# edantec/MPC_benchmark

Hardware: AMD Instinct MI355X
Metric: mpc_solves_per_sec (higher is better)
Workload: dtype f64

## Files before the change

### mpc_benchmark_amd/csrc/legs.h

```cpp
#pragma once
#include "mfma_blocks.h"
#include "solver_kernels.h"

#define LEG_BARRIER() asm volatile("s_waitcnt lgkmcnt(0)\n\ts_barrier" ::: "memory")

#define LEG_LAUNDER() do { asm volatile("" : "+v"(tid), "+v"(lane)); wv = __builtin_amdgcn_readfirstlane(tid >> 6); } while (0)

#define LK_THREADS 512
#define LK_U 20
#define LK_PT 13
#define LK_TILES 5

struct LkLds {
  int np, mp, nzp, lda, ldp, ldm, nb, nbm;
  int AB, PR, TM, ZN, vec, total_bytes;
  unsigned mg_nzp, mg_np, mg_mp;
};
static inline constexpr LkLds make_lk_lds(int n, int m) {
  LkLds s{};
  s.np = (n + 15) & ~15; s.mp = (m + 15) & ~15; s.nzp = s.np + s.mp; s.lda = s.nzp + 1; s.ldp = s.np + 1; s.ldm = s.mp + 1;
  s.nb = s.np / 16; s.nbm = s.mp / 16;
  s.mg_nzp = magic_div(s.nzp); s.mg_np = magic_div(s.np); s.mg_mp = magic_div(s.mp);
  int o = 0;
  auto take = [&](int cnt) { int r = o; o += (cnt + 1) & ~1; return r; };
// ... 733 lines not shown
  constexpr int FW_ROWS = NP / 8;
  for (int j = 0; j + 1 < J; ++j) {
    double* lr = leg_ptr(a, b, j);
    const int cut = leg_start(a, j + 1);
    const int c0 = lane < n ? lane : 0, c1 = lane + 64 < n ? lane + 64 : 0;
    const double m0 = lane < n ? 1.0 : 0.0, m1 = lane + 64 < n ? 1.0 : 0.0;
    double va[FW_ROWS][2];
    if (j > 0) {
#pragma unroll
      for (int i = 0; i < FW_ROWS; ++i) { const int r = wv + i * nw, rr = r < n ? r : 0; va[i][0] = lr[L.lZx + rr * n + c0] * m0; va[i][1] = lr[L.lZx + rr * n + c1] * m1; }
    }
#pragma unroll
    for (int i = 0; i < FW_ROWS; ++i) {
      const int r = wv + i * nw;
      double sx = 0.0;
      if (j > 0) sx = wave_sum(va[i][0] * xv[c0] + va[i][1] * xv[c1]);
      if (lane == 0 && r < n) { ev[r] = sx + lr[L.lzc + r]; a.dxs[((size_t)b * (N + 1) + cut) * n + r] = ev[r]; }
    }
#pragma unroll
    for (int i = 0; i < FW_ROWS; ++i) { const int r = wv + i * nw, rr = r < n ? r : 0; va[i][0] = lr[L.ldP + rr * n + c0] * m0; va[i][1] = lr[L.ldP + rr * n + c1] * m1; }
    LEG_BARRIER();
#pragma unroll
    for (int i = 0; i < FW_ROWS; ++i) {
      const int r = wv + i * nw;
      const double sx = wave_sum(va[i][0] * ev[c0] + va[i][1] * ev[c1]);
      if (lane == 0 && r < n) lr[L.lth + r] = sx + lr[L.lcp + r];
    }
    for (int i = tid; i < n; i += nthr) xv[i] = ev[i];
    LEG_BARRIER();
  }
  LEG_PROF(29);
}

__global__ void __launch_bounds__(256) k_leg_apply(SolverArgs a) {
  const Layout& L = a.L;
  const int k = blockIdx.x, b = blockIdx.y, tid = threadIdx.x, nthr = blockDim.x, lane = tid & 63, wv = tid >> 6, nw = nthr >> 6;
  const InstState& st = a.inst[b];
  if (st.done || st.skip_step) return;
  const int j = leg_of_knot(a, k);
  if (j + 1 >= a.nlegs) return;
  const int n = L.n, ke = leg_start(a, j + 1) - 1;
  const double* kn = knot_ptr(a, b, k);
  double* g = gain_ptr(a, b, k);
  const int m = (int)kn[L.oMISC + MISC_M], c = (int)kn[L.oMISC + MISC_NC];
  const double* th_g = leg_ptr(a, b, j) + L.lth;
  __shared__ double th[128], pn[128];
  __shared__ int act_idx[256];
  __shared__ int wcnt[4];
  for (int i = tid; i < n; i += nthr) th[i] = th_g[i];
  const bool is_act = tid < c && kn[L.oACT + (tid < c ? tid : 0)] != 0.0;
  const unsigned long long amask = __ballot(is_act);
  if (lane == 0) wcnt[wv] = __popcll(amask);
  __syncthreads();
  int ca = 0;
  {
    int off = 0;
    for (int q = 0; q < nw; ++q) { if (q < wv) off += wcnt[q]; ca += wcnt[q]; }
    if (is_act) act_idx[off + __popcll(amask & ((1ull << lane) - 1ull))] = tid;
  }
  const int c0 = lane < n ? lane : 0, c1 = lane + 64 < n ? lane + 64 : 0;
  const double m0 = lane < n ? 1.0 : 0.0, m1 = lane + 64 < n ? 1.0 : 0.0;
  if (k == ke) { for (int i = tid; i < n; i += nthr) pn[i] = th[i]; }
  else {
    const double* gn = gain_ptr(a, b, k + 1) + L.oLm;
    const double t0 = th[c0] * m0, t1 = th[c1] * m1;
    for (int r0 = 4 * wv; r0 < n; r0 += 4 * nw) {
      double v[4][2];
#pragma unroll
      for (int q = 0; q < 4; ++q) { const int r = r0 + q < n ? r0 + q : 0; v[q][0] = gn[r * n + c0]; v[q][1] = gn[r * n + c1]; }
#pragma unroll
      for (int q = 0; q < 4; ++q) { const double sx = wave_sum(v[q][0] * t0 + v[q][1] * t1); if (lane == 0 && r0 + q < n) pn[r0 + q] = sx; }
    }
  }
  __syncthreads();
  const double t0 = th[c0] * m0, t1 = th[c1] * m1, q0 = pn[c0] * m0, q1 = pn[c1] * m1;
  const int total = 2 * n + m + ca;
  for (int r0 = 4 * wv; r0 < total; r0 += 4 * nw) {
    double v[4][2];
    double* dst[4];
    bool use_th[4];
#pragma unroll
    for (int q = 0; q < 4; ++q) {
      const int r = r0 + q < total ? r0 + q : 0;
      const double* row;
      if (r < n) { row = g + L.oLm + r * n; dst[q] = g + L.op + r; use_th[q] = true; }
      else if (r < 2 * n) { row = g + L.oGam + (r - n) * n; dst[q] = g + L.ophi + (r - n); use_th[q] = false; }
      else if (r < 2 * n + m) { row = g + L.oKu + (r - 2 * n) * n; dst[q] = g + L.ok + (r - 2 * n); use_th[q] = false; }
      else { row = g + L.oKnup + (r - 2 * n - m) * n; dst[q] = g + L.oknu + act_idx[r - 2 * n - m]; use_th[q] = false; }
      v[q][0] = row[c0]; v[q][1] = row[c1];
    }
#pragma unroll
    for (int q = 0; q < 4; ++q) {
      const double sx = wave_sum(use_th[q] ? v[q][0] * t0 + v[q][1] * t1 : v[q][0] * q0 + v[q][1] * q1);
      if (lane == 0 && r0 + q < total) *dst[q] += sx;
    }
  }
}
```

### mpc_benchmark_amd/csrc/mpc_hip.hip

```cpp
#include <hip/hip_runtime.h>
#include <mutex>
#include <map>
#include <cmath>
#include <cstdio>
#include <cstdlib>
#include <cstring>
#include <limits>
#include <stdexcept>
#include <string>
#include <utility>
#include <vector>

#include "eval_multibody_host.h"
#include "eval_reuse_kernels.h"
#include "eval_vector.h"
#include "riccati_mfma.h"
#include "closed_loop.h"
#include "legs.h"
#include "legs_tree.h"
#include "pipeline_glue.h"
#include "pipeline_ikid_glue.h"
#include "pipeline_contacts.h"
#include "pipeline_fd_glue.h"
#include "sim_record.h"
// ... 134 lines not shown
  size_t d_patch_cap = 0;
  double* h_xnext[2] = {nullptr, nullptr};
  std::vector<double> leg_mu;
  static constexpr int ASYNC_DEPTH = 2;
  InstState* h_status[ASYNC_DEPTH] = {nullptr, nullptr};
  hipEvent_t status_ev[ASYNC_DEPTH] = {nullptr, nullptr};
  int async_head = 0, async_pending = 0;
  static constexpr int STAGE_RING = 8;
  char* stage_pin[STAGE_RING] = {};
  hipEvent_t stage_ev[STAGE_RING] = {};
  int stage_next = 0;
  RicLds ric{};
  int ric_fixed = 0;
  ClLds cl{};
  bool use_mfma_riccati = false;
  LkLds lk{};
  LcLds lc{};
  LxLds lx{};
  bool legs_ok = false;
  bool env_chain = false, env_plain = false, env_reject_failed = false;
  int env_tree_sweeps = 0, env_trace = -1;
  int env_tail_knots = -1, cu_count = 0;
  int tail_last = 0, tail_sweeps_last = 0;
  long long tail_fused = 0, tail_separate = 0;
  long long leg_passes_multi = 0, leg_passes_single = 0;
  int leg_tail_knots(int J) const {
    if (J < 2 || env_tail_knots == 0) return 0;
    const int last = L.N - (int)((long long)(J - 1) * L.N / J);
    if (env_tail_knots > 0) return env_tail_knots < last ? env_tail_knots : last;
    if ((long long)J * L.B > cu_count || (long long)L.N * L.B <= cu_count) return 0;
    const int t = 21 * (L.N / J) / 25;
    return t < last ? t : last;
  }
  double* d_legbuf = nullptr;
  double* d_treebuf = nullptr;
  int leg_cap = 0;
  TreeDesc tree{};
  bool use_tree() const {
    return eff_legs() >= 3 && d_treebuf != nullptr && !env_chain;
  }
  bool leg_guess_valid = false;
  int leg_guess_now = 0;
  int eff_legs() const {
    if (!legs_ok) return 1;
    int J = opt.riccati_legs;
    if (J > MPC_MAX_LEGS) J = MPC_MAX_LEGS;
    if (J > L.N) J = L.N;
    return J < 1 ? 1 : J;
  }
  struct ProfSlot {
    const char* name;
    std::vector<std::pair<hipEvent_t, hipEvent_t>> ev;
    size_t used = 0;
  };
  bool profiling = false;
  unsigned prof_mask = ~0u;
  std::vector<ProfSlot> prof;

  template <class F> void timed(int slot, const char* name, F&& launch) {
    if (!profiling || !((prof_mask >> slot) & 1u) || pass_is_corrector) { launch(); return; }
    if ((int)prof.size() <= slot) prof.resize(slot + 1);
    ProfSlot& p = prof[slot];
    p.name = name;
    if (p.used == p.ev.size()) {
      hipEvent_t e0, e1;
      HIP_OK(hipEventCreate(&e0));
// ... 48 lines not shown
}

static void ensure_leg_capacity(mpc_solver* s, int legs) {
  const Layout& L = s->L;
  int need = legs < 1 ? 1 : legs;
  if (need >= 3 && need < 4) need = 4;
  if (need <= s->leg_cap) return;
  HIP_OK(hipStreamSynchronize(s->stream));
  auto regrow = [&](double*& p, size_t count) {
    if (p) HIP_OK(hipFree(p));
    p = nullptr;
    HIP_OK(hipMalloc((void**)&p, (count ? count : 1) * sizeof(double)));
    HIP_OK(hipMemsetAsync(p, 0, (count ? count : 1) * sizeof(double), s->stream));
  };
  const size_t B = L.B;
  regrow(s->d_work, B * need * (size_t)L.work_stride);
  if (s->legs_ok) {
    regrow(s->d_legbuf, B * (size_t)(need > 1 ? need - 1 : 1) * L.leg_stride);
    regrow(s->d_treebuf, B * (size_t)need * L.tree_stride);
  }
  s->leg_cap = need;
  s->leg_guess_valid = false;
  HIP_OK(hipStreamSynchronize(s->stream));
}

static void create_impl(mpc_solver* s, const mpc_dims& d) {
  s->dims = d;
  { const char* e;
    e = getenv("MPC_LEGS_CHAIN"); s->env_chain = e && atoi(e) > 0;
    e = getenv("MPC_LEGS_PLAIN"); s->env_plain = e && atoi(e) > 0;
    e = getenv("MPC_HIP_REJECT_FAILED"); s->env_reject_failed = e && atoi(e) > 0;
    e = getenv("MPC_TREE_SWEEPS"); s->env_tree_sweeps = e ? atoi(e) : 0;
    e = getenv("MPC_HIP_TRACE"); s->env_trace = e ? atoi(e) : -1;
    e = getenv("MPC_LEG_TAIL_KNOTS"); s->env_tail_knots = e ? (atoi(e) > 0 ? atoi(e) : 0) : -1; }
  HIP_OK(hipSetDevice(d.device));
  HIP_OK(hipDeviceGetAttribute(&s->cu_count, hipDeviceAttributeMultiprocessorCount, d.device));
  { const char* e = getenv("MPC_LEG_TAIL_CUS"); if (e && atoi(e) > 0) s->cu_count = atoi(e); }
  {
    static int created = 0;
    const char* pe = getenv("MPC_HIP_STREAM_PRIO");
    if (pe && atoi(pe) > 0) {
      int lo = 0, hi = 0;
      HIP_OK(hipDeviceGetStreamPriorityRange(&lo, &hi));
      const int levels = lo - hi + 1;
      const int prio = hi + (created++ % levels);
      HIP_OK(hipStreamCreateWithPriority(&s->stream, hipStreamNonBlocking, prio));
      if (atoi(pe) > 1) fprintf(stderr, "[mpc] stream priority %d (range %d..%d)\n", prio, hi, lo);
    } else {
      HIP_OK(hipStreamCreateWithFlags(&s->stream, hipStreamNonBlocking));
    }
  }
  Layout& L = s->L;
  L.N = d.horizon; L.B = d.batch; L.space = d.space; L.nx = d.nx; L.n = d.ndx; L.m = d.nu; L.c = d.nc_max > 0 ? d.nc_max : 1;
  L.nj = 0;
  L.max_stage_ints = d.max_stage_ints; L.max_stage_doubles = d.max_stage_doubles;
  L.n_alpha = 8;
  make_layout(L);
  Layout& T = s->LT;
  T = L;
  {
    int o = 0;
    auto take = [&](int cnt) { int r = o; o += align2(cnt); return r; };
    T.oCV = take(L.c); T.oCT = take(L.c); T.oLO = take(L.c); T.oHI = take(L.c); T.oDT = take(L.c); T.oACT = take(L.c);
    T.oF = take(L.n); T.oMISC = take(MISC_COUNT);
    T.oH = T.oG = T.oAB = T.oE6 = T.oT6k = T.oD12 = T.oCD = T.oXD = T.oWR = T.oXN = 0;
    T.knot_stride = o;
  }
// ... 379 lines not shown
        case 48: MPC_TREE_LAUNCH(48); break;
        case 64: MPC_TREE_LAUNCH(64); break;
        default: MPC_TREE_LAUNCH(80); break;
      }
#undef MPC_TREE_LAUNCH
    });
    if (tree) s->timed(16, "k_leg_tree_down", [&] {
      const TreeDesc& T = s->tree;
      if (false) {
#define X(ID, FN, FM, GF, ST, NPV, MPV) } else if (s->ric_fixed == ID) { for (int lev = T.nlev - 1; lev >= 0; --lev) hipLaunchKernelGGL((k_leg_tree_down<NPV, FN, FM>), dim3(T.lev_cnt[lev] + (lev == T.nlev - 1 ? 1 : 0), L.B), dim3(LK_THREADS), s->lx.total_bytes, s->stream, a, s->lx, T, lev);
      MPC_FIXED_MODELS(X)
#undef X
      } else switch (s->lx.np) {
        case 16: for (int lev = T.nlev - 1; lev >= 0; --lev) hipLaunchKernelGGL(k_leg_tree_down<16>, dim3(T.lev_cnt[lev] + (lev == T.nlev - 1 ? 1 : 0), L.B), dim3(LK_THREADS), s->lx.total_bytes, s->stream, a, s->lx, T, lev); break;
        case 32: for (int lev = T.nlev - 1; lev >= 0; --lev) hipLaunchKernelGGL(k_leg_tree_down<32>, dim3(T.lev_cnt[lev] + (lev == T.nlev - 1 ? 1 : 0), L.B), dim3(LK_THREADS), s->lx.total_bytes, s->stream, a, s->lx, T, lev); break;
        case 48: for (int lev = T.nlev - 1; lev >= 0; --lev) hipLaunchKernelGGL(k_leg_tree_down<48>, dim3(T.lev_cnt[lev] + (lev == T.nlev - 1 ? 1 : 0), L.B), dim3(LK_THREADS), s->lx.total_bytes, s->stream, a, s->lx, T, lev); break;
        case 64: for (int lev = T.nlev - 1; lev >= 0; --lev) hipLaunchKernelGGL(k_leg_tree_down<64>, dim3(T.lev_cnt[lev] + (lev == T.nlev - 1 ? 1 : 0), L.B), dim3(LK_THREADS), s->lx.total_bytes, s->stream, a, s->lx, T, lev); break;
        default: for (int lev = T.nlev - 1; lev >= 0; --lev) hipLaunchKernelGGL(k_leg_tree_down<80>, dim3(T.lev_cnt[lev] + (lev == T.nlev - 1 ? 1 : 0), L.B), dim3(LK_THREADS), s->lx.total_bytes, s->stream, a, s->lx, T, lev); break;
      }
    });
    else s->timed(14, "k_leg_consensus", [&] {
      switch (s->lx.np) {
        case 16: hipLaunchKernelGGL(k_leg_consensus<16>, dim3(L.B), dim3(LK_THREADS), s->lx.total_bytes, s->stream, a, s->lx); break;
        case 32: hipLaunchKernelGGL(k_leg_consensus<32>, dim3(L.B), dim3(LK_THREADS), s->lx.total_bytes, s->stream, a, s->lx); break;
        case 48: hipLaunchKernelGGL(k_leg_consensus<48>, dim3(L.B), dim3(LK_THREADS), s->lx.total_bytes, s->stream, a, s->lx); break;
        case 64: hipLaunchKernelGGL(k_leg_consensus<64>, dim3(L.B), dim3(LK_THREADS), s->lx.total_bytes, s->stream, a, s->lx); break;
        default: hipLaunchKernelGGL(k_leg_consensus<80>, dim3(L.B), dim3(LK_THREADS), s->lx.total_bytes, s->stream, a, s->lx); break;
      }
    });
  }
  }
  if (J > 1) {
    s->leg_guess_valid = true;
    s->timed(15, "k_leg_apply", [&] { hipLaunchKernelGGL(k_leg_apply, dim3(L.N, L.B), dim3(256), 0, s->stream, a); });
    s->timed(4, "k_forward", [&] {
      if (L.m <= 32) hipLaunchKernelGGL((k_forward_phi<4, 10>), dim3(L.B * J), dim3(512), 2 * L.n * sizeof(double), s->stream, a);
      else hipLaunchKernelGGL((k_forward_phi<6, 10>), dim3(L.B * J), dim3(512), 2 * L.n * sizeof(double), s->stream, a);
    });
  } else {
  const bool fw_phi = s->cl.total_bytes <= 160 * 1024 && L.n <= 80 && L.m <= 32 && (s->opt.forward_mode == 0 ? L.B * L.N <= 2048 : s->opt.forward_mode == 2);
  if (fw_phi) {
    s->timed(12, "k_closed_loop", [&] { hipLaunchKernelGGL(k_closed_loop, dim3(L.N, L.B), dim3(CL_THREADS), s->cl.total_bytes, s->stream, a, s->cl); });
    s->timed(4, "k_forward", [&] { hipLaunchKernelGGL((k_forward_phi<4, 10>), dim3(L.B), dim3(512), 2 * L.n * sizeof(double), s->stream, a); });
  } else {
    s->timed(4, "k_forward", [&] {
      const size_t fw_lds = (L.nz + 2 * L.n) * sizeof(double);
      const bool fits = L.nz <= 128 && L.n + L.m <= L.nz;
      if (fits && L.n <= 80 && L.m <= 48) a.abdz = s->d_abdz;
      if (fits && L.n <= 80 && L.m <= 32) hipLaunchKernelGGL((k_forward_prefetch<4, 10>), dim3(L.B), dim3(512), fw_lds, s->stream, a);
      else if (fits && L.n <= 80 && L.m <= 48) hipLaunchKernelGGL((k_forward_prefetch<6, 10>), dim3(L.B), dim3(512), fw_lds, s->stream, a);
      else hipLaunchKernelGGL(k_forward, dim3(L.B), dim3(1024), fw_lds, s->stream, a);
    });
  }
  }
  s->timed(5, "k_duals", [&] { hipLaunchKernelGGL(k_duals, dim3(L.N + 1, L.B), dim3(256), (L.nz + 3 * L.n + 16 + 3 * L.c) * sizeof(double), s->stream, a); });
  if (a.spec_on || L.space != MPC_SPACE_MULTIBODY) s->timed(6, "k_eval_stage_trial", [&] { launch_eval(s, true, 0, 1, a.spec_on != 0); });
  else s->timed(17, "k_eval_stage_trial_values", [&] { launch_eval(s, true, 0, 1, false); });
  s->spec_rec_valid = a.spec_on != 0 && a.spec_knot != nullptr;
  s->timed(7, "k_linesearch", [&] { hipLaunchKernelGGL(k_linesearch, dim3(L.B), dim3(64), 0, s->stream, a, 1, 0); });
  const int nc1 = (L.n_alpha - 1 < 2 || (size_t)L.B * (L.N + 1) < 2048) ? L.n_alpha - 1 : 2;
  s->timed(10, "k_eval_stage_backtrack", [&] { launch_eval(s, true, 1, nc1); });
  s->timed(11, "k_linesearch_backtrack", [&] { hipLaunchKernelGGL(k_linesearch, dim3(L.B), dim3(64), 0, s->stream, a, 0, nc1); });
  if (L.n_alpha - 1 - nc1 > 0) {
    s->timed(10, "k_eval_stage_backtrack", [&] { launch_eval(s, true, 1 + nc1, L.n_alpha - 1 - nc1); });
    s->timed(11, "k_linesearch_backtrack", [&] { hipLaunchKernelGGL(k_linesearch, dim3(L.B), dim3(64), 0, s->stream, a, 0, L.n_alpha); });
  }
  s->timed(8, "k_accept", [&] { hipLaunchKernelGGL(k_accept, dim3(L.N + 1, L.B), dim3(64), 0, s->stream, a); });
  s->timed(9, "k_after_step", [&] { hipLaunchKernelGGL(k_after_step, dim3(L.B), dim3(1), 0, s->stream, a); });
  HIP_OK(hipGetLastError());
}

static void report_status(mpc_solver* s, int B, const InstState* st, mpc_stats* stats) {
  for (int b = 0; b < B; ++b) {
    if (st[b].done >= 2) s->leg_guess_valid = false;
    if (st[b].done >= 2 && !s->isolate) throw std::runtime_error("Riccati factorisation failed on instance " + std::to_string(b) + " (code " + std::to_string(st[b].done) + ")");
    if (!stats) continue;
    mpc_stats& o = stats[b];
    o.num_iters = st[b].num_iters; o.converged = st[b].done >= 2 ? -st[b].done : st[b].converged; o.al_iters = st[b].al_iters; o.ls_steps = st[b].ls_step;
    o.traj_cost = st[b].cost; o.merit = st[b].phi0; o.prim_infeas = st[b].prim; o.dual_infeas = st[b].dual; o.mu = st[b].mu; o.alpha = st[b].alpha;
  }
}

static void begin_refine(mpc_solver* s) {
  s->refine_now = s->L.N >= 1 && ((s->opt.refine_appended_knot > 0 && s->appended_changed) || (s->opt.refine_appended_knot < 0 && s->appended_any));
  s->appended_changed = false; s->appended_any = false;
  if (s->refine_now) { s->slot_dirty[slot_of(s, s->L.N - 1)] = 1; s->slot_dirty[s->L.N] = 1; }
}
static void launch_refine(mpc_solver* s) {
// ... 378 lines not shown
#define X(ID, FN, FM, GF, ST, NPV, MPV) else if (s->ric_fixed == ID) e.push_back({"k_riccati_mfma<512,80,true,true," #FN "," #FM "," #GF "," #ST "> (sweep, legs, fixed dimensions)", (const void*)k_riccati_mfma<RIC_THREADS, 80, true, true, FN, FM, GF, ST>, RIC_THREADS, s->ric.total_bytes, (long long)L.B * J});
      MPC_FIXED_MODELS(X)
#undef X
      else if (s->ric.sq) e.push_back({"k_riccati_mfma<512,80,true,true> (sweep, legs)", (const void*)k_riccati_mfma<RIC_THREADS, 80, true, true>, RIC_THREADS, s->ric.total_bytes, (long long)L.B * J});
      else e.push_back({"k_riccati_mfma<512,80,false,true> (sweep, legs)", (const void*)k_riccati_mfma<RIC_THREADS, 80, false, true>, RIC_THREADS, s->ric.total_bytes, (long long)L.B * J});
      const void* lk = s->lk.mp <= 16 ? (const void*)k_leg_knot<16> : (s->lk.mp <= 32 ? (const void*)k_leg_knot<32> : (const void*)k_leg_knot<48>);
      const void* lcd = (const void*)k_leg_condense<0>;
      const void* lct = s->lk.mp <= 16 ? (const void*)k_leg_condense_tail<16> : (s->lk.mp <= 32 ? (const void*)k_leg_condense_tail<32> : (const void*)k_leg_condense_tail<48>);
      const char* lct_name = "k_leg_condense_tail (condensation + the last leg's knots)";
      const char *lk_name = "k_leg_knot", *lcd_name = "k_leg_condense", *lcmp_name = "k_leg_compose (first level of the tree over the cuts)", *ltd_name = "k_leg_tree_down (last level)";
      const void *lcmp_fixed = nullptr, *ltd_fixed = nullptr;
#define X(ID, FN, FM, GF, ST, NPV, MPV) if (s->ric_fixed == ID) { lk = (const void*)k_leg_knot<MPV, FN, FM>; lcd = (const void*)k_leg_condense<FN>; lct = (const void*)k_leg_condense_tail<MPV, FN, FM>; lct_name = "k_leg_condense_tail<" #MPV "," #FN "," #FM "> (fixed dimensions)"; lcmp_fixed = (const void*)k_leg_compose<NPV, FN, FM>; ltd_fixed = (const void*)k_leg_tree_down<NPV, FN, FM>; \
        lk_name = "k_leg_knot<" #MPV "," #FN "," #FM "> (fixed dimensions)"; lcd_name = "k_leg_condense<" #FN "> (fixed dimensions)"; \
        lcmp_name = "k_leg_compose<" #NPV "," #FN "," #FM "> (first level of the tree over the cuts, fixed dimensions)"; ltd_name = "k_leg_tree_down<" #NPV "," #FN "," #FM "> (last level, fixed dimensions)"; }
      MPC_FIXED_MODELS(X)
#undef X
      const int tail = s->leg_tail_knots(J);
      e.push_back({lk_name, lk, LK_THREADS, s->lk.total_bytes, (long long)(L.N - tail) * L.B});
      if (tail > 0) e.push_back({lct_name, lct, LK_THREADS, s->lc.total_bytes > s->lk.total_bytes ? s->lc.total_bytes : s->lk.total_bytes, (long long)J * L.B});
      else e.push_back({lcd_name, lcd, LK_THREADS, s->lc.total_bytes, (long long)(J - 1) * L.B});
      if (s->use_tree()) {
        const TreeDesc T = make_tree_desc(J);
        const void* lc = s->lx.np == 16 ? (const void*)k_leg_compose<16> : s->lx.np == 32 ? (const void*)k_leg_compose<32> : s->lx.np == 48 ? (const void*)k_leg_compose<48>
                       : s->lx.np == 64 ? (const void*)k_leg_compose<64> : (const void*)k_leg_compose<80>;
        const void* ld = s->lx.np == 16 ? (const void*)k_leg_tree_down<16> : s->lx.np == 32 ? (const void*)k_leg_tree_down<32> : s->lx.np == 48 ? (const void*)k_leg_tree_down<48>
                       : s->lx.np == 64 ? (const void*)k_leg_tree_down<64> : (const void*)k_leg_tree_down<80>;
        e.push_back({lcmp_name, lcmp_fixed ? lcmp_fixed : lc, LCMP_THREADS, s->lx.total_bytes, (long long)(T.lev_cnt[0] + 1) * L.B * 2});
        e.push_back({ltd_name, ltd_fixed ? ltd_fixed : ld, LK_THREADS, s->lx.total_bytes, (long long)T.lev_cnt[0] * L.B});
      } else {
      const void* lx = s->lx.np == 16 ? (const void*)k_leg_consensus<16> : s->lx.np == 32 ? (const void*)k_leg_consensus<32> : s->lx.np == 48 ? (const void*)k_leg_consensus<48>
                     : s->lx.np == 64 ? (const void*)k_leg_consensus<64> : (const void*)k_leg_consensus<80>;
      e.push_back({"k_leg_consensus", lx, LK_THREADS, s->lx.total_bytes, (long long)L.B});
      }
      e.push_back({"k_leg_apply", (const void*)k_leg_apply, 256, 0, (long long)L.N * L.B});
      e.push_back({"k_forward_phi (forward sweeps of the legs)", L.m <= 32 ? (const void*)k_forward_phi<4, 10> : (const void*)k_forward_phi<6, 10>, 512, (int)(2 * L.n * sizeof(double)), (long long)L.B * J});
    } else if (s->use_mfma_riccati) {
      const void* fn = small ? (const void*)k_riccati_mfma<RIC_SMALL_THREADS, 16> : (s->ric.sq && s->ric.np <= 80) ? (const void*)k_riccati_mfma<RIC_THREADS, 80, true>
                     : s->ric.sq ? (const void*)k_riccati_mfma<RIC_THREADS, 96, true> : s->ric.np <= 80 ? (const void*)k_riccati_mfma<RIC_THREADS, 80> : (const void*)k_riccati_mfma<RIC_THREADS, 96>;
      e.push_back({"k_riccati_mfma (serial sweep)", fn, small ? RIC_SMALL_THREADS : RIC_THREADS, s->ric.total_bytes, (long long)L.B});
    } else e.push_back({"k_riccati_backward (serial sweep, no matrix cores)", (const void*)k_riccati_backward, 256, (int)s->riccati_lds(), (long long)L.B});
    e.push_back({"k_duals", (const void*)k_duals, 256, (int)((L.nz + 3 * L.n + 16 + 3 * L.c) * sizeof(double)), (long long)(L.N + 1) * L.B});
    e.push_back({"k_lagrangian", (const void*)k_lagrangian, 64, 0, (long long)(L.N + 1) * L.B});
    if (idx < 0 || idx >= (int)e.size()) return (int)e.size();
    const Ent& k = e[idx];
    hipFuncAttributes at;
    HIP_OK(hipFuncGetAttributes(&at, k.fn));
    int nb = 0;
    HIP_OK(hipOccupancyMaxActiveBlocksPerMultiprocessor(&nb, k.fn, k.block, (size_t)k.dyn));
    if (name && name_cap > 0) { strncpy(name, k.name, name_cap - 1); name[name_cap - 1] = 0; }
    info[0] = k.block; info[1] = at.numRegs; info[2] = (int)at.localSizeBytes; info[3] = (int)at.sharedSizeBytes; info[4] = k.dyn; info[5] = nb;
    info[6] = (int)k.grid; info[7] = nb * ((k.block + 63) / 64) / 4;
    return (int)e.size();
  } catch (const std::exception& ex) { s->err = ex.what(); return -1; }
}

int mpc_profile_read(mpc_solver* s, int32_t slot, char* name, int32_t name_cap, int32_t* launches, double* total_ms) {
  if (!s) return -2;
  try {
    HIP_OK(hipSetDevice(s->dims.device));
    HIP_OK(hipStreamSynchronize(s->stream));
    const int nslots = (int)s->prof.size();
    if (slot < 0 || slot >= nslots) return nslots;
    const mpc_solver::ProfSlot& p = s->prof[slot];
    double tot = 0;
    for (size_t i = 0; i < p.used; ++i) {
      float ms = 0;
      HIP_OK(hipEventElapsedTime(&ms, p.ev[i].first, p.ev[i].second));
      tot += ms;
    }
    if (name && name_cap > 0) { std::strncpy(name, p.name ? p.name : "", name_cap - 1); name[name_cap - 1] = 0; }
    if (launches) *launches = (int32_t)p.used;
    if (total_ms) *total_ms = tot;
    return nslots;
  } catch (const std::exception& e) {
// ... 365 lines not shown
    else if (nm == "Knu") { for (int i = 0; i < c; ++i) if (kn[L.oACT + i] == 0.0) for (int z = 0; z < n; ++z) g[L.oKnu + i * n + z] = 0.0; mat(g.data() + L.oKnu, c, n, n); }
    else if (nm == "knu") mat(g.data() + L.oknu, 1, c, c);
    else if (nm == "Mx") mat(g.data() + L.oMx, k < L.N ? n : 0, n, n);
    else if (nm == "mx") mat(g.data() + L.omx, 1, k < L.N ? n : 0, n);
    else if (nm == "Phi") mat(g.data() + L.oPhi, k < L.N ? n : 0, n, n);
    else if (nm == "phi") mat(g.data() + L.ophi, 1, k < L.N ? n : 0, n);
    else if (nm == "Gam") mat(g.data() + L.oGam, n, n, n);
    else if (nm == "Ku") mat(g.data() + L.oKu, m, n, n);
    else if (nm == "Lm") mat(g.data() + L.oLm, n, n, n);
    else if (nm == "Mu") mat(g.data() + L.oMu, m, m, L.mpad);
    else if (nm == "Znu" || nm == "Knup") {
      const bool zn = nm == "Znu";
      const int cols = zn ? m : n, ld = zn ? L.mpad : n;
      v.assign((size_t)c * cols, 0.0);
      int ai = 0;
      for (int i = 0; i < c; ++i) if (kn[L.oACT + i] != 0.0) { for (int j = 0; j < cols; ++j) v[(size_t)i * cols + j] = g[(zn ? L.oZnu : L.oKnup) + ai * ld + j]; ++ai; }
    }
    else if (nm == "Sg" || nm == "sg" || nm == "Zx" || nm == "zc" || nm == "calP" || nm == "calp" || nm == "theta") {
      if (!s->d_legbuf || k >= s->leg_cap - 1) throw std::runtime_error("debug_get: no such leg record");
      const double* lr = s->d_legbuf + ((size_t)b * (s->leg_cap - 1) + k) * L.leg_stride;
      if (nm == "Sg") dev_vec(lr + L.lSg, n * n); else if (nm == "sg") dev_vec(lr + L.lsg, n); else if (nm == "Zx") dev_vec(lr + L.lZx, n * n);
      else if (nm == "zc") dev_vec(lr + L.lzc, n); else if (nm == "calP") dev_vec(lr + L.ldP, n * n);
      else if (nm == "calp") dev_vec(lr + L.lcp, n);
      else dev_vec(lr + L.lth, n);
    }
    else if (nm == "ls_knot") {
      std::vector<double> tp((size_t)L.n_alpha * (L.N + 1));
      copy_sync(s, tp.data(), s->d_trial_phi + (size_t)b * L.n_alpha * (L.N + 1), tp.size() * sizeof(double), hipMemcpyDeviceToHost);
      for (int i = 0; i < L.n_alpha; ++i) v.push_back(tp[(size_t)i * (L.N + 1) + k]);
      v.push_back(kn[L.oMISC + MISC_COST]); v.push_back(kn[L.oMISC + MISC_PEN]);
    }
    else if (nm == "leg_tail") v = {(double)s->tail_last, (double)s->tail_fused, (double)s->tail_separate, (double)s->tail_sweeps_last, (double)s->eff_legs(), (double)s->cu_count,
                                   (double)s->leg_passes_multi, (double)s->leg_passes_single};
    else if (nm == "fixed_dims") v = {(double)s->ric_fixed};
    else if (nm == "ric_prof") { dev_vec(s->d_prof + (size_t)b * 64, 64); HIP_OK(hipMemsetAsync(s->d_prof + (size_t)b * 64, 0, 64 * sizeof(double), s->stream)); HIP_OK(hipStreamSynchronize(s->stream)); }
    else if (nm == "dx") dev_vec(s->d_dxs + ((size_t)b * (L.N + 1) + k) * n, n);
    else if (nm == "du") { if (k >= L.N) throw std::runtime_error("no du at the terminal knot"); dev_vec(s->d_dus + ((size_t)b * L.N + k) * L.m, L.m); }
    else if (nm == "dvs") dev_vec(s->d_dvs + ((size_t)b * (L.N + 1) + k) * L.c, L.c);
    else if (nm == "dlams") dev_vec(s->d_dlams + ((size_t)b * (L.N + 1) + k) * n, n);
    else throw std::runtime_error("debug_get: unknown quantity " + nm);
    if ((int)v.size() > cap) throw std::runtime_error("debug_get: output buffer too small");
    if (!v.empty()) std::memcpy(out, v.data(), v.size() * sizeof(double));
    return (int)v.size();
  } catch (const std::exception& e) {
    s->err = e.what();
    return -1;
  }
}

}

#include "walk_poses.h"
#include "walk_commands.h"
#include "sim_host.h"
#include "pipeline_loops.h"
```

### mpc_benchmark_amd/csrc/solver_kernels.h

```cpp
#pragma once
#include "solver_args.h"


__global__ void k_lagrangian(SolverArgs a) {
  const Layout& L = a.L;
  const int k = blockIdx.x, b = blockIdx.y, tid = threadIdx.x, nthr = blockDim.x;
  const InstState& st = a.inst[b];
  if (st.done) return;
  double* kn = knot_ptr(a, b, k);
  const int n = L.n, nz = L.nz, N = L.N;
  const int c = (int)kn[L.oMISC + MISC_NC], m = (int)kn[L.oMISC + MISC_M], nzk = n + m;
  const double mu = st.mu, mud = mu * a.opt.dyn_al_scale;
  const double* v = a.vs + ((size_t)b * (N + 1) + k) * L.c;
  const double* lamn = a.lams + ((size_t)b * (N + 1) + k + 1) * n;
  const double* lamk = a.lams + ((size_t)b * (N + 1) + k) * n;
  __shared__ double red[64];
  double dual = 0.0, crit = 0.0;
  for (int z = tid; z < nzk; z += nthr) {
    double s = kn[L.oG + z];
    for (int i = 0; i < c; ++i) if (v[i] != 0.0) s += kn[L.oCD + i * nz + z] * v[i];
    if (k < N) for (int i = 0; i < n; ++i) if (lamn[i] != 0.0) s += kn[L.oAB + i * nz + z] * lamn[i];
    if (k > 0 && z < n) {
      if (L.space == MPC_SPACE_MULTIBODY && z < 6) {
        const double* E6 = knot_ptr(a, b, k - 1) + L.oE6;
// ... 401 lines not shown
#pragma unroll
    for (int q = 0; q < FW_NR; ++q) {
      const int r = wv + nw * q;
      if (r < n) {
        double s = (c0 < n + m ? ABr[q][0] * dz[c0] : 0.0) + (c1 < n + m ? ABr[q][1] * dz[c1] : 0.0);
        s = wave_sum(s);
        if (lane == 0) { y[r] = s + mxv[q]; if (a.abdz) a.abdz[((size_t)b * N + k) * n + r] = s; }
      }
    }
    if (more) load_AB(k + 1);
    FW_BARRIER();
#pragma unroll
    for (int q = 0; q < FW_NR; ++q) {
      const int r = wv + nw * q;
      if (r < n) {
        double s = (c0 < n ? Mr[q][0] * y[c0] : 0.0) + (c1 < n ? Mr[q][1] * y[c1] : 0.0);
        s = wave_sum(s);
        if (lane == 0) z[r] = y[r] - mud * s;
      }
    }
    if (more) load_M(k + 1);
    FW_BARRIER();
    if (tid < n) {
      double s = z[tid];
      if (ff && tid < 6) { s = 0; for (int l = 0; l < 6; ++l) s += t6[l] * z[l]; }
      dz[tid] = s;
      a.dxs[((size_t)b * (N + 1) + k + 1) * n + tid] = s;
    }
    if (more) load_T6(k + 1);
    FW_BARRIER();
  }
}

__global__ void __launch_bounds__(256) k_duals(SolverArgs a) {
  const Layout& L = a.L;
  const int k = blockIdx.x, b = blockIdx.y, tid = threadIdx.x, nthr = blockDim.x, lane = tid & 63, wv = tid >> 6, nw = nthr >> 6;
  const InstState& st = a.inst[b];
  if (st.done || st.skip_step) return;
  const int n = L.n, nz = L.nz, N = L.N;
  double* kn = knot_ptr(a, b, k);
  const double* g = gain_ptr(a, b, k);
  const int c = (int)kn[L.oMISC + MISC_NC], m = (int)kn[L.oMISC + MISC_M];
  const double mu = st.mu, mud = mu * a.opt.dyn_al_scale;
  const bool ff = L.space == MPC_SPACE_MULTIBODY;
  const double* v = a.vs + ((size_t)b * (N + 1) + k) * L.c;
  double* dv = a.dvs + ((size_t)b * (N + 1) + k) * L.c;
  extern __shared__ __attribute__((aligned(16))) double sh[];
  double* dz = sh;
  double* dxn = dz + nz;
  double* lnew = dxn + n;
  double* jdl = lnew + n;
  double* part = jdl + n;
  for (int z = tid; z < n + m; z += nthr) dz[z] = (z < n) ? a.dxs[((size_t)b * (N + 1) + k) * n + z] : a.dus[((size_t)b * N + k) * L.m + z - n];
  if (k < N) for (int z = tid; z < n; z += nthr) dxn[z] = a.dxs[((size_t)b * (N + 1) + k + 1) * n + z];
  __syncthreads();
  double* rsc = part + nw + 2;
  for (int i = tid; i < L.c; i += nthr) {
    const bool in = i < c;
    rsc[i] = in ? kn[L.oACT + i] : 0.0; rsc[L.c + i] = in ? kn[L.oDT + i] / mu : 0.0; rsc[2 * L.c + i] = in ? v[i] : 0.0;
  }
  __syncthreads();
  double acc = 0.0;
  if (wv == 0) {
    double s = 0;
    for (int z = lane; z < n + m; z += 64) s += kn[L.oG + z] * dz[z];
    acc += wave_sum(s);
  }
  for (int i = wv; i < L.c; i += nw) {
    if (i >= c) { if (lane == 0) dv[i] = 0.0; continue; }
    double s = 0, jd = 0;
    const bool act = rsc[i] != 0.0;
    const double vp = rsc[L.c + i], vi = rsc[2 * L.c + i];
    const double wj = vp + (act ? (vp - vi) : 0.0);
    if (act)
      for (int z = lane; z < n; z += 64) s += g[L.oKnu + i * n + z] * dz[z];
    if (wj != 0.0)
      for (int z = lane; z < n + m; z += 64) jd += kn[L.oCD + i * nz + z] * dz[z];
    s = wave_sum(s) + g[L.oknu + i];
    jd = wave_sum(jd);
    const double dvi = s - vi;
    if (lane == 0) dv[i] = dvi;
    acc += wj * jd - mu * (vp - vi) * dvi;
  }
  if (k == 0) for (int i = tid; i < n; i += nthr) a.dlams[(size_t)b * (N + 1) * n + i] = 0.0;
  if (k < N) {
    const double* gn = gain_ptr(a, b, k + 1);
    const bool have = a.abdz != nullptr;
    const int c0 = lane < n ? lane : 0, c1 = lane + 64 < n ? lane + 64 : 0;
    const double d0 = lane < n ? dxn[c0] : 0.0, d1 = lane + 64 < n ? dxn[c1] : 0.0;
    if (n > 128) {
      for (int i = wv; i < n; i += nw) {
        double s = 0;
        for (int z = lane; z < n; z += 64) s += gn[L.oP + i * n + z] * dxn[z];
        s = wave_sum(s);
        if (lane == 0) { lnew[i] = s + gn[L.op + i]; jdl[i] = have ? a.abdz[((size_t)b * N + k) * n + i] : 0.0; }
      }
    } else
    for (int r0 = 4 * wv; r0 < n; r0 += 4 * nw) {
      double pv[4][2];
#pragma unroll
      for (int q = 0; q < 4; ++q) { const int r = r0 + q < n ? r0 + q : 0; pv[q][0] = gn[L.oP + r * n + c0]; pv[q][1] = gn[L.oP + r * n + c1]; }
#pragma unroll
      for (int q = 0; q < 4; ++q) {
        const int i = r0 + q;
        const double s = wave_sum(pv[q][0] * d0 + pv[q][1] * d1);
        if (lane == 0 && i < n) { lnew[i] = s + gn[L.op + i]; jdl[i] = have ? a.abdz[((size_t)b * N + k) * n + i] : 0.0; }
      }
    }
  }
  if (lane == 0) part[wv] = acc;
  __syncthreads();
  if (k < N && wv == 0) {
// ... 303 lines not shown
```

Before: 12180.

## Chunk leg-apply over several knots per block and stage duals knu offsets

k_leg_apply now processes a chunk of C consecutive knots per block instead of one knot per block. It computes all the propagated theta products for the chunk in one pass with double-buffered loads that overlap global reads with wave reductions. Launch count drops when batch times horizon exceeds the CU count. k_duals becomes templated: the default path preloads the knu offsets into shared memory and skips wave reductions for inactive constraints. In exchange the kernels use more dynamic LDS and have fewer blocks for latency hiding.

```diff
diff --git a/mpc_benchmark_amd/csrc/legs.h b/mpc_benchmark_amd/csrc/legs.h
--- a/mpc_benchmark_amd/csrc/legs.h
+++ b/mpc_benchmark_amd/csrc/legs.h
@@ -789,67 +789,118 @@
   LEG_PROF(29);
 }
 
-__global__ void __launch_bounds__(256) k_leg_apply(SolverArgs a) {
+#define LEG_APPLY_MAX_CHUNK 32
+static inline size_t leg_apply_lds(int n, int C) {
+  return (size_t)(C + 2) * n * sizeof(double) + (size_t)C * (4 * sizeof(unsigned long long) + 2 * sizeof(int) + 256 * sizeof(unsigned short));
+}
+static inline int leg_apply_chunks(int N, int J, int C) {
+  int t = 0;
+  for (int j = 0; j + 1 < J; ++j) t += ((int)((long long)(j + 1) * N / J) - (int)((long long)j * N / J) + C - 1) / C;
+  return t;
+}
+struct LegApplyBatch { double v[4][2]; double old[4]; int kk, r0; };
+template <class Rows, class Load, class Reduce>
+DEV void leg_apply_rows(int count, int wv, Rows&& rows_of, Load&& load, Reduce&& reduce) {
+  int kk = 0, r0 = 4 * wv;
+  auto settle = [&] { while (kk < count && r0 >= rows_of(kk)) { ++kk; r0 = 4 * ((wv + kk) & 3); } };
+  auto next = [&](LegApplyBatch& t) { r0 += 16; settle(); if (kk >= count) return false; t.kk = kk; t.r0 = r0; load(t); return true; };
+  settle();
+  if (kk >= count) return;
+  LegApplyBatch x, y;
+  x.kk = kk; x.r0 = r0; load(x);
+  for (;;) {
+    bool more = next(y);
+    reduce(x);
+    if (!more) break;
+    more = next(x);
+    reduce(y);
+    if (!more) break;
+  }
+}
+__global__ void __launch_bounds__(256) k_leg_apply(SolverArgs a, int C) {
   const Layout& L = a.L;
-  const int k = blockIdx.x, b = blockIdx.y, tid = threadIdx.x, nthr = blockDim.x, lane = tid & 63, wv = tid >> 6, nw = nthr >> 6;
+  const int b = blockIdx.y, tid = threadIdx.x, lane = tid & 63, wv = tid >> 6;
   const InstState& st = a.inst[b];
   if (st.done || st.skip_step) return;
-  const int j = leg_of_knot(a, k);
-  if (j + 1 >= a.nlegs) return;
-  const int n = L.n, ke = leg_start(a, j + 1) - 1;
-  const double* kn = knot_ptr(a, b, k);
-  double* g = gain_ptr(a, b, k);
-  const int m = (int)kn[L.oMISC + MISC_M], c = (int)kn[L.oMISC + MISC_NC];
+  int x = blockIdx.x, j = 0, k0 = 0, ke = -1;
+  for (; j + 1 < a.nlegs; ++j) {
+    const int s0 = leg_start(a, j), s1 = leg_start(a, j + 1), nc = (s1 - s0 + C - 1) / C;
+    if (x < nc) { k0 = s0 + x * C; ke = s1 - 1; break; }
+    x -= nc;
+  }
+  if (ke < 0) return;
+  const int n = L.n, cn = ke - k0 + 1 < C ? ke - k0 + 1 : C;
+  const bool at_end = k0 + cn - 1 == ke;
+  const int nq = at_end ? cn : cn + 1;
+  extern __shared__ __attribute__((aligned(16))) double la_sh[];
+  double* th = la_sh;
+  double* qv = th + n;
+  unsigned long long* amask_s = (unsigned long long*)(qv + (size_t)(C + 1) * n);
+  int* mm = (int*)(amask_s + 4 * C);
+  int* cas = mm + C;
+  unsigned short* act_idx = (unsigned short*)(cas + C);
   const double* th_g = leg_ptr(a, b, j) + L.lth;
-  __shared__ double th[128], pn[128];
-  __shared__ int act_idx[256];
-  __shared__ int wcnt[4];
-  for (int i = tid; i < n; i += nthr) th[i] = th_g[i];
-  const bool is_act = tid < c && kn[L.oACT + (tid < c ? tid : 0)] != 0.0;
-  const unsigned long long amask = __ballot(is_act);
-  if (lane == 0) wcnt[wv] = __popcll(amask);
+  double* g0 = gain_ptr(a, b, k0);
+  const size_t gs = L.gain_stride;
+  for (int i = tid; i < n; i += 256) th[i] = th_g[i];
+  for (int kk = 0; kk < cn; ++kk) {
+    const double* kn = knot_ptr(a, b, k0 + kk);
+    const int c = (int)kn[L.oMISC + MISC_NC];
+    const bool is_act = tid < c && kn[L.oACT + (tid < c ? tid : 0)] != 0.0;
+    const unsigned long long am = __ballot(is_act);
+    if (lane == 0) amask_s[4 * kk + wv] = am;
+    if (tid == 0) mm[kk] = (int)kn[L.oMISC + MISC_M];
+  }
   __syncthreads();
-  int ca = 0;
-  {
-    int off = 0;
-    for (int q = 0; q < nw; ++q) { if (q < wv) off += wcnt[q]; ca += wcnt[q]; }
-    if (is_act) act_idx[off + __popcll(amask & ((1ull << lane) - 1ull))] = tid;
+  for (int kk = 0; kk < cn; ++kk) {
+    int off = 0, ca = 0;
+    for (int w = 0; w < 4; ++w) { const int pc = __popcll(amask_s[4 * kk + w]); if (w < wv) off += pc; ca += pc; }
+    const unsigned long long am = amask_s[4 * kk + wv];
+    if ((am >> lane) & 1ull) act_idx[256 * kk + off + __popcll(am & ((1ull << lane) - 1ull))] = (unsigned short)tid;
+    if (tid == 0) cas[kk] = ca;
   }
   const int c0 = lane < n ? lane : 0, c1 = lane + 64 < n ? lane + 64 : 0;
   const double m0 = lane < n ? 1.0 : 0.0, m1 = lane + 64 < n ? 1.0 : 0.0;
-  if (k == ke) { for (int i = tid; i < n; i += nthr) pn[i] = th[i]; }
-  else {
-    const double* gn = gain_ptr(a, b, k + 1) + L.oLm;
+  {
     const double t0 = th[c0] * m0, t1 = th[c1] * m1;
-    for (int r0 = 4 * wv; r0 < n; r0 += 4 * nw) {
-      double v[4][2];
-#pragma unroll
-      for (int q = 0; q < 4; ++q) { const int r = r0 + q < n ? r0 + q : 0; v[q][0] = gn[r * n + c0]; v[q][1] = gn[r * n + c1]; }
-#pragma unroll
-      for (int q = 0; q < 4; ++q) { const double sx = wave_sum(v[q][0] * t0 + v[q][1] * t1); if (lane == 0 && r0 + q < n) pn[r0 + q] = sx; }
-    }
+    if (at_end) for (int i = tid; i < n; i += 256) qv[cn * n + i] = th[i];
+    leg_apply_rows(nq, wv, [&](int) { return n; },
+      [&](LegApplyBatch& t) {
+        const double* gn = g0 + t.kk * gs + L.oLm;
+#pragma unroll
+        for (int q = 0; q < 4; ++q) { const int r = t.r0 + q < n ? t.r0 + q : 0; t.v[q][0] = gn[r * n + c0]; t.v[q][1] = gn[r * n + c1]; }
+      },
+      [&](const LegApplyBatch& t) {
+#pragma unroll
+        for (int q = 0; q < 4; ++q) { const double sx = wave_sum(__builtin_fma(t.v[q][0], t0, t.v[q][1] * t1)); if (lane == 0 && t.r0 + q < n) qv[t.kk * n + t.r0 + q] = sx; }
+      });
   }
   __syncthreads();
-  const double t0 = th[c0] * m0, t1 = th[c1] * m1, q0 = pn[c0] * m0, q1 = pn[c1] * m1;
-  const int total = 2 * n + m + ca;
-  for (int r0 = 4 * wv; r0 < total; r0 += 4 * nw) {
-    double v[4][2];
-    double* dst[4];
-    bool use_th[4];
-#pragma unroll
-    for (int q = 0; q < 4; ++q) {
-      const int r = r0 + q < total ? r0 + q : 0;
-      const double* row;
-      if (r < n) { row = g + L.oLm + r * n; dst[q] = g + L.op + r; use_th[q] = true; }
-      else if (r < 2 * n) { row = g + L.oGam + (r - n) * n; dst[q] = g + L.ophi + (r - n); use_th[q] = false; }
-      else if (r < 2 * n + m) { row = g + L.oKu + (r - 2 * n) * n; dst[q] = g + L.ok + (r - 2 * n); use_th[q] = false; }
-      else { row = g + L.oKnup + (r - 2 * n - m) * n; dst[q] = g + L.oknu + act_idx[r - 2 * n - m]; use_th[q] = false; }
-      v[q][0] = row[c0]; v[q][1] = row[c1];
-    }
-#pragma unroll
-    for (int q = 0; q < 4; ++q) {
-      const double sx = wave_sum(use_th[q] ? v[q][0] * t0 + v[q][1] * t1 : v[q][0] * q0 + v[q][1] * q1);
-      if (lane == 0 && r0 + q < total) *dst[q] += sx;
-    }
-  }
-}
+  for (int idx = tid; idx < cn * n; idx += 256) { const int kk = idx / n; g0[kk * gs + L.op + (idx - kk * n)] += qv[idx]; }
+  auto dst_of = [&](int kk, int r) -> double* {
+    double* g = g0 + kk * gs;
+    const int m = mm[kk];
+    return r < n ? g + L.ophi + r : (r < n + m ? g + L.ok + (r - n) : g + L.oknu + act_idx[256 * kk + (r - n - m)]);
+  };
+  leg_apply_rows(cn, wv, [&](int kk) { return n + mm[kk] + cas[kk]; },
+    [&](LegApplyBatch& t) {
+      double* g = g0 + t.kk * gs;
+      const int m = mm[t.kk], total = n + m + cas[t.kk];
+#pragma unroll
+      for (int q = 0; q < 4; ++q) {
+        const int r = t.r0 + q < total ? t.r0 + q : 0;
+        const double* row = r < n ? g + L.oGam + r * n : (r < n + m ? g + L.oKu + (r - n) * n : g + L.oKnup + (r - n - m) * n);
+        t.v[q][0] = row[c0]; t.v[q][1] = row[c1];
+        t.old[q] = *dst_of(t.kk, r);
+      }
+    },
+    [&](const LegApplyBatch& t) {
+      const int total = n + mm[t.kk] + cas[t.kk];
+      const double q0 = qv[(t.kk + 1) * n + c0] * m0, q1 = qv[(t.kk + 1) * n + c1] * m1;
+#pragma unroll
+      for (int q = 0; q < 4; ++q) {
+        const double sx = wave_sum(__builtin_fma(t.v[q][0], q0, t.v[q][1] * q1));
+        if (lane == 0 && t.r0 + q < total) *dst_of(t.kk, t.r0 + q) = t.old[q] + sx;
+      }
+    });
+}
diff --git a/mpc_benchmark_amd/csrc/mpc_hip.hip b/mpc_benchmark_amd/csrc/mpc_hip.hip
--- a/mpc_benchmark_amd/csrc/mpc_hip.hip
+++ b/mpc_benchmark_amd/csrc/mpc_hip.hip
@@ -190,6 +190,17 @@
     const int t = 21 * (L.N / J) / 25;
     return t < last ? t : last;
   }
+  int env_apply_chunk = -1;
+  bool env_duals_plain = false;
+  int apply_chunk_last = 0;
+  long long apply_chunked = 0, apply_single = 0;
+  long long duals_staged = 0, duals_plain = 0;
+  int leg_apply_chunk(int J) const {
+    int C;
+    if (env_apply_chunk > 0) C = env_apply_chunk;
+    else C = (long long)L.N * L.B <= cu_count ? 1 : 5;
+    return C < 1 ? 1 : (C > LEG_APPLY_MAX_CHUNK ? LEG_APPLY_MAX_CHUNK : C);
+  }
   double* d_legbuf = nullptr;
   double* d_treebuf = nullptr;
   int leg_cap = 0;
@@ -304,7 +315,9 @@
     e = getenv("MPC_HIP_REJECT_FAILED"); s->env_reject_failed = e && atoi(e) > 0;
     e = getenv("MPC_TREE_SWEEPS"); s->env_tree_sweeps = e ? atoi(e) : 0;
     e = getenv("MPC_HIP_TRACE"); s->env_trace = e ? atoi(e) : -1;
-    e = getenv("MPC_LEG_TAIL_KNOTS"); s->env_tail_knots = e ? (atoi(e) > 0 ? atoi(e) : 0) : -1; }
+    e = getenv("MPC_LEG_TAIL_KNOTS"); s->env_tail_knots = e ? (atoi(e) > 0 ? atoi(e) : 0) : -1;
+    e = getenv("MPC_LEG_APPLY_CHUNK"); s->env_apply_chunk = (e && atoi(e) > 0) ? atoi(e) : -1;
+    e = getenv("MPC_DUALS_PLAIN"); s->env_duals_plain = e && atoi(e) > 0; }
   HIP_OK(hipSetDevice(d.device));
   HIP_OK(hipDeviceGetAttribute(&s->cu_count, hipDeviceAttributeMultiprocessorCount, d.device));
   { const char* e = getenv("MPC_LEG_TAIL_CUS"); if (e && atoi(e) > 0) s->cu_count = atoi(e); }
@@ -750,7 +763,12 @@
   }
   if (J > 1) {
     s->leg_guess_valid = true;
-    s->timed(15, "k_leg_apply", [&] { hipLaunchKernelGGL(k_leg_apply, dim3(L.N, L.B), dim3(256), 0, s->stream, a); });
+    s->timed(15, "k_leg_apply", [&] {
+      const int C = s->leg_apply_chunk(J);
+      s->apply_chunk_last = C;
+      if (C > 1) s->apply_chunked++; else s->apply_single++;
+      hipLaunchKernelGGL(k_leg_apply, dim3(leg_apply_chunks(L.N, J, C), L.B), dim3(256), leg_apply_lds(L.n, C), s->stream, a, C);
+    });
     s->timed(4, "k_forward", [&] {
       if (L.m <= 32) hipLaunchKernelGGL((k_forward_phi<4, 10>), dim3(L.B * J), dim3(512), 2 * L.n * sizeof(double), s->stream, a);
       else hipLaunchKernelGGL((k_forward_phi<6, 10>), dim3(L.B * J), dim3(512), 2 * L.n * sizeof(double), s->stream, a);
@@ -771,7 +789,10 @@
     });
   }
   }
-  s->timed(5, "k_duals", [&] { hipLaunchKernelGGL(k_duals, dim3(L.N + 1, L.B), dim3(256), (L.nz + 3 * L.n + 16 + 3 * L.c) * sizeof(double), s->stream, a); });
+  s->timed(5, "k_duals", [&] {
+    if (s->env_duals_plain) { s->duals_plain++; hipLaunchKernelGGL(k_duals<true>, dim3(L.N + 1, L.B), dim3(256), (L.nz + 3 * L.n + 16 + 3 * L.c) * sizeof(double), s->stream, a); }
+    else { s->duals_staged++; hipLaunchKernelGGL(k_duals<false>, dim3(L.N + 1, L.B), dim3(256), (L.nz + 3 * L.n + 16 + 4 * L.c) * sizeof(double), s->stream, a); }
+  });
   if (a.spec_on || L.space != MPC_SPACE_MULTIBODY) s->timed(6, "k_eval_stage_trial", [&] { launch_eval(s, true, 0, 1, a.spec_on != 0); });
   else s->timed(17, "k_eval_stage_trial_values", [&] { launch_eval(s, true, 0, 1, false); });
   s->spec_rec_valid = a.spec_on != 0 && a.spec_knot != nullptr;
@@ -1216,14 +1237,16 @@
                      : s->lx.np == 64 ? (const void*)k_leg_consensus<64> : (const void*)k_leg_consensus<80>;
       e.push_back({"k_leg_consensus", lx, LK_THREADS, s->lx.total_bytes, (long long)L.B});
       }
-      e.push_back({"k_leg_apply", (const void*)k_leg_apply, 256, 0, (long long)L.N * L.B});
+      { const int C = s->leg_apply_chunk(J);
+        e.push_back({"k_leg_apply", (const void*)k_leg_apply, 256, (int)leg_apply_lds(L.n, C), (long long)leg_apply_chunks(L.N, J, C) * L.B}); }
       e.push_back({"k_forward_phi (forward sweeps of the legs)", L.m <= 32 ? (const void*)k_forward_phi<4, 10> : (const void*)k_forward_phi<6, 10>, 512, (int)(2 * L.n * sizeof(double)), (long long)L.B * J});
     } else if (s->use_mfma_riccati) {
       const void* fn = small ? (const void*)k_riccati_mfma<RIC_SMALL_THREADS, 16> : (s->ric.sq && s->ric.np <= 80) ? (const void*)k_riccati_mfma<RIC_THREADS, 80, true>
                      : s->ric.sq ? (const void*)k_riccati_mfma<RIC_THREADS, 96, true> : s->ric.np <= 80 ? (const void*)k_riccati_mfma<RIC_THREADS, 80> : (const void*)k_riccati_mfma<RIC_THREADS, 96>;
       e.push_back({"k_riccati_mfma (serial sweep)", fn, small ? RIC_SMALL_THREADS : RIC_THREADS, s->ric.total_bytes, (long long)L.B});
     } else e.push_back({"k_riccati_backward (serial sweep, no matrix cores)", (const void*)k_riccati_backward, 256, (int)s->riccati_lds(), (long long)L.B});
-    e.push_back({"k_duals", (const void*)k_duals, 256, (int)((L.nz + 3 * L.n + 16 + 3 * L.c) * sizeof(double)), (long long)(L.N + 1) * L.B});
+    if (s->env_duals_plain) e.push_back({"k_duals<true> (MPC_DUALS_PLAIN)", (const void*)k_duals<true>, 256, (int)((L.nz + 3 * L.n + 16 + 3 * L.c) * sizeof(double)), (long long)(L.N + 1) * L.B});
+    else e.push_back({"k_duals", (const void*)k_duals<false>, 256, (int)((L.nz + 3 * L.n + 16 + 4 * L.c) * sizeof(double)), (long long)(L.N + 1) * L.B});
     e.push_back({"k_lagrangian", (const void*)k_lagrangian, 64, 0, (long long)(L.N + 1) * L.B});
     if (idx < 0 || idx >= (int)e.size()) return (int)e.size();
     const Ent& k = e[idx];
@@ -1655,6 +1678,8 @@
     }
     else if (nm == "leg_tail") v = {(double)s->tail_last, (double)s->tail_fused, (double)s->tail_separate, (double)s->tail_sweeps_last, (double)s->eff_legs(), (double)s->cu_count,
                                    (double)s->leg_passes_multi, (double)s->leg_passes_single};
+    else if (nm == "backsubst") v = {(double)s->apply_chunk_last, (double)s->apply_chunked, (double)s->apply_single, (double)s->duals_staged, (double)s->duals_plain,
+                                    (double)leg_apply_chunks(L.N, s->eff_legs(), s->apply_chunk_last > 0 ? s->apply_chunk_last : 1)};
     else if (nm == "fixed_dims") v = {(double)s->ric_fixed};
     else if (nm == "ric_prof") { dev_vec(s->d_prof + (size_t)b * 64, 64); HIP_OK(hipMemsetAsync(s->d_prof + (size_t)b * 64, 0, 64 * sizeof(double), s->stream)); HIP_OK(hipStreamSynchronize(s->stream)); }
     else if (nm == "dx") dev_vec(s->d_dxs + ((size_t)b * (L.N + 1) + k) * n, n);
diff --git a/mpc_benchmark_amd/csrc/solver_kernels.h b/mpc_benchmark_amd/csrc/solver_kernels.h
--- a/mpc_benchmark_amd/csrc/solver_kernels.h
+++ b/mpc_benchmark_amd/csrc/solver_kernels.h
@@ -457,6 +457,7 @@
   }
 }
 
+template <bool PLAIN>
 __global__ void __launch_bounds__(256) k_duals(SolverArgs a) {
   const Layout& L = a.L;
   const int k = blockIdx.x, b = blockIdx.y, tid = threadIdx.x, nthr = blockDim.x, lane = tid & 63, wv = tid >> 6, nw = nthr >> 6;
@@ -483,6 +484,7 @@
   for (int i = tid; i < L.c; i += nthr) {
     const bool in = i < c;
     rsc[i] = in ? kn[L.oACT + i] : 0.0; rsc[L.c + i] = in ? kn[L.oDT + i] / mu : 0.0; rsc[2 * L.c + i] = in ? v[i] : 0.0;
+    if (!PLAIN) rsc[3 * L.c + i] = in ? g[L.oknu + i] : 0.0;
   }
   __syncthreads();
   double acc = 0.0;
@@ -501,8 +503,13 @@
       for (int z = lane; z < n; z += 64) s += g[L.oKnu + i * n + z] * dz[z];
     if (wj != 0.0)
       for (int z = lane; z < n + m; z += 64) jd += kn[L.oCD + i * nz + z] * dz[z];
-    s = wave_sum(s) + g[L.oknu + i];
-    jd = wave_sum(jd);
+    if (PLAIN) {
+      s = wave_sum(s) + g[L.oknu + i];
+      jd = wave_sum(jd);
+    } else {
+      if (act || wj != 0.0) { s = wave_sum(s); jd = wave_sum(jd); }
+      s = s + rsc[3 * L.c + i];
+    }
     const double dvi = s - vi;
     if (lane == 0) dv[i] = dvi;
     acc += wj * jd - mu * (vp - vi) * dvi;
```

After: 12310, median of 6. 1.1% higher.
